# martingoe/physics

Measured on AMD Instinct MI355X. Metric: rigid_body_steps_per_sec, higher is better.
Workload: dtype f32; 1 GPU; C5_256000_tower; n_bodies=256000, bodies_per_gpu=256000, dt_nanos=16666667, preroll_steps=30, rccl_ranks=0

## Files before the change

include/spec/contact_solve.h:

```cpp
#ifndef PHYS_SPEC_CONTACT_SOLVE_H
#define PHYS_SPEC_CONTACT_SOLVE_H

#include "collide.h"

#define PHYS_MAX_COLORS 64
#define PHYS_COLOR_CACHE_PERIOD 64
#define PHYS_WARM_DIST 0.05f
#define PHYS_WARM_DOT 0.999f

typedef struct {
    float dt;
    float baumgarte;
    float slop;
    float friction;
    float max_bias;
} solve_params_t;

typedef struct {
    v3 rA, rB;
    float normal_mass;
    float tangent_mass[2];
    float bias;
    float pn;
    float pt[2];
// ... 253 lines not shown
            }
        }
    }
}

typedef struct {
    v3 n, t1, t2;
    int count;
    int has_b;
    v3 pt[4];
    float bias[4];
    float pn[4], pt0[4], pt1[4];
    float mass[4][3];
} geo_manifold_t;

PHYS_HD void solve_manifold_geo(geo_manifold_t* gm, int make_masses, int apply_only, float friction, v3 xA, float invMA, const m33* IA,
                                v3 xB, float invMB, const m33* IB, v3* vA, v3* wA, v3* vB, v3* wB) {
    const v3 zero = v3_make(0.0f, 0.0f, 0.0f);
    const int has_b = gm->has_b;
    v3 lA[3], lB[3];
    PHYS_UNROLL
    for (int d = 0; d < 3; ++d) {
        const v3 dir = d == 0 ? gm->t1 : (d == 1 ? gm->t2 : gm->n);
        lA[d] = v3_scale(dir, invMA);
        lB[d] = has_b ? v3_scale(dir, invMB) : zero;
    }
    PHYS_UNROLL
    for (int k = 0; k < 4; ++k) {
        if (k < gm->count) {
            const v3 rA = v3_sub(gm->pt[k], xA);
            const v3 rB = has_b ? v3_sub(gm->pt[k], xB) : zero;
            PHYS_UNROLL
            for (int t = 0; t < 3; ++t) {
                const v3 dir = t == 0 ? gm->t1 : (t == 1 ? gm->t2 : gm->n);
                jac_row_t j;
                j.aA = v3_cross_f(rA, dir);
                j.mA = inertia_mul(IA, j.aA);
                if (has_b) {
                    j.aB = v3_cross_f(rB, dir);
                    j.mB = inertia_mul(IB, j.aB);
                } else {
                    j.aB = zero; j.mB = zero;
                }
                if (make_masses) {
                    float km = invMA + v3_dot_f(j.mA, j.aA);
                    if (has_b) km = (km + invMB) + v3_dot_f(j.mB, j.aB);
                    gm->mass[k][t] = km > 0.0f ? 1.0f / km : 0.0f;
                }
                if (apply_only) {
                    row_apply(t == 0 ? gm->pt0[k] : (t == 1 ? gm->pt1[k] : gm->pn[k]), lA[t], lB[t], &j, has_b, vA, wA, vB, wB);
                    continue;
                }
                const float mass = gm->mass[k][t];
                const float vrel = row_velocity(dir, &j, has_b, *vA, *wA, *vB, *wB);
                float lambda;
                if (t < 2) {
                    float* acc = t == 0 ? &gm->pt0[k] : &gm->pt1[k];
                    lambda = -mass * vrel;
                    const float maxf = friction * gm->pn[k];
                    const float old = *acc;
                    const float np = det_maxf(-maxf, det_minf(old + lambda, maxf));
                    lambda = np - old;
                    *acc = np;
                } else {
                    lambda = mass * (gm->bias[k] - vrel);
                    const float old = gm->pn[k];
                    const float np = det_maxf(old + lambda, 0.0f);
                    lambda = np - old;
                    gm->pn[k] = np;
                }
                row_apply(lambda, lA[t], lB[t], &j, has_b, vA, wA, vB, wB);
            }
        }
    }
}

#endif
```

physics_amd/csrc/abi.hip:

```cpp
#include <algorithm>
#include <atomic>
#include <cmath>
#include <cstdlib>
#include <cstring>
#include <limits>
#include <string>
#include <vector>

#include "kernels.hpp"

namespace phys {
static thread_local std::string g_error;
void set_error(const std::string& msg) { g_error = msg; }
const char* get_error() { return g_error.c_str(); }
}

using namespace phys;

namespace phys {
void poll_snapshots(phys_world* w);
StepCounters* snapshot_acquire(phys_world* w) {
    const uint32_t k = w->snap_next;
    if (w->snap_pending[k]) {
        (void)hipEventSynchronize(w->snap_event[k]);
// ... 449 lines not shown

static int32_t fetch_counters(phys_world* w) {
    PHYS_HIP_TRY(hipMemcpyAsync(w->h_counters, w->counters.p, sizeof(StepCounters), hipMemcpyDeviceToHost, w->stream));
    PHYS_HIP_TRY(hipStreamSynchronize(w->stream));
    return PHYS_OK;
}

int32_t phys_sync(phys_world* w) {
    ENTER(w);
    const int32_t rc = fetch_counters(w);
    if (rc != PHYS_OK) return rc;
    poll_snapshots(w);
    const uint32_t bits = w->h_counters->overflow | w->h_counters->sticky_overflow | w->host_sticky_overflow;
    if (w->h_counters->n_static_pairs > w->static_pairs_seen) w->static_pairs_seen = w->h_counters->n_static_pairs;
    w->host_sticky_overflow = 0;
    if (w->h_counters->sticky_overflow) {
        PHYS_HIP_TRY(hipMemsetAsync(&w->counters.p->sticky_overflow, 0, sizeof(uint32_t), w->stream));
        PHYS_HIP_TRY(hipStreamSynchronize(w->stream));
    }
    if (bits & kOvfCorruptRow) {
        const uint32_t* g = w->h_counters->debug;
        return fail(PHYS_ERR_HIP, ("internal error: a solver row names no body of this world and was refused (row " +
                                   std::to_string(g[0]) + ": a " + std::to_string(g[1]) + ", b " + std::to_string(g[2]) + ", points " +
                                   std::to_string(g[3]) + "; colour " + std::to_string(g[6]) + " rows [" + std::to_string(g[4]) + ", " +
                                   std::to_string(g[5]) + "), tile base " + std::to_string(g[7]) + ")").c_str());
    }
    if (w->h_counters->debug[0] != 0u) {
        PHYS_HIP_TRY(hipMemsetAsync(w->counters.p->debug, 0, sizeof(w->counters.p->debug), w->stream));
        PHYS_HIP_TRY(hipStreamSynchronize(w->stream));
    }
    if ((bits & kOvfHandoff) && w->h_counters->debug[0] == 0xC1u) {
        const uint32_t* g = w->h_counters->debug;
        return fail(PHYS_ERR_HIP, ("contact solver hand-off timed out (k_solve_cluster) in a step since the last phys_sync; velocities "
                                   "are invalid from that step on. First lane to give up: cluster " + std::to_string(g[1] & 0xFFFFu) + " of " + std::to_string(g[1] >> 16) + ", row " +
                                   std::to_string(g[2]) + ", bodies " + std::to_string(g[3]) + " / " + std::to_string(g[4]) +
                                   ", tickets " + std::to_string(g[5] & 0xFFFFu) + " / " + std::to_string(g[5] >> 16) + ", waiting A/B " +
                                   std::to_string(g[6] & 1u) + "/" + std::to_string((g[6] >> 1) & 1u) + ", modes " +
                                   std::to_string((g[6] >> 4) & 3u) + "/" + std::to_string((g[6] >> 8) & 3u) + ", iteration " +
                                   std::to_string((g[7] >> 8) & 0xFFu) + ", colour " + std::to_string(g[7] & 0xFFu) +
                                   ". If other work shares this GPU with phys_update, create the world WITHOUT PHYS_FLAG_EXCLUSIVE_GPU").c_str());
    }
    if (bits & kOvfHandoff)
        return fail(PHYS_ERR_HIP, "contact solver hand-off timed out (k_solve_flow) in a step since the last phys_sync; "
                                  "velocities are invalid from that step on");
    if (bits & kOvfColors)
        return fail(PHYS_ERR_CAPACITY, "a body has more than 64 contact manifolds (PHYS_MAX_COLORS): the contact solve of "
                                       "that step was skipped. This limit is not configurable");
    if (bits & kOvfHalo)
        return fail(PHYS_ERR_CAPACITY, "halo record / cross-pair capacity exceeded in a step since the last phys_sync");
    if (bits & kOvfColorTable)
        return fail(PHYS_ERR_CAPACITY, "the persistent colour table is full (a look-up or an insert gave up after thousands of "
                                       "slots): the contact solve of that step was skipped. Raise phys_config.max_manifolds");
    if (bits)
        return fail(PHYS_ERR_CAPACITY, "pair / manifold capacity exceeded in a step since the last phys_sync (the contact "
                                       "solve of that step was skipped): raise phys_config.max_pairs / max_manifolds");
    return PHYS_OK;
}

static int32_t d2h(phys_world* w, void* dst, const void* src, size_t bytes) {
// ... 506 lines not shown
```

physics_amd/csrc/cluster.hip:

```cpp
#include <algorithm>
#include <cstdio>
#include <cstdlib>
#include <mutex>
#include <vector>

#include "kernels.hpp"

namespace phys {

constexpr int kClusterPerCuDiag = 3, kClusterPerCuFull = 2;
constexpr size_t kClusterLdsPerCu = 160 * 1024;
constexpr size_t kClusterSlotBytesDecl = 64;
size_t cluster_lds_bytes(uint32_t slots);

__host__ __device__ __forceinline__ uint32_t side_info(uint32_t slot, uint32_t mode) { return (slot & 0x3FFFu) | (mode << 14); }

static uint32_t spread10(uint32_t x) {
    x &= 0x3ffu;
    x = (x ^ (x << 16)) & 0xff0000ffu;
    x = (x ^ (x << 8)) & 0x0300f00fu;
    x = (x ^ (x << 4)) & 0x030c30c3u;
    x = (x ^ (x << 2)) & 0x09249249u;
    return x;
}

static size_t seg_count_offset(uint64_t n) { return ((size_t)2 * n + 3) & ~(size_t)3; }

static uint32_t clusters_on_chip(int per_cu, int cus) { return (uint32_t)std::max(8, per_cu * (cus - cus / 8)); }

int32_t cluster_assign(phys_world* w, const float* pos ) {
    w->cluster_count = 0;
    w->seg_count_dirty = false;
    w->seg_count_bins = 0;
    const uint64_t n = w->n, n_owned = w->n_owned;
    const DebugSwitches& dbg = debug_switches();
    w->cluster_dynamic = false;
    w->cluster_homes_valid = false;
    if (dbg.no_cluster || n_owned < kClusterMinBodies || !w->flow_vel.p) return PHYS_OK;
    int cus = 0;
    PHYS_HIP_TRY(hipDeviceGetAttribute(&cus, hipDeviceAttributeMultiprocessorCount, w->device));
    w->cluster_cus = cus;
    const int per_cu_max = w->all_diag_inertia ? kClusterPerCuDiag : kClusterPerCuFull;
    int per_cu = dbg.clusters_per_cu ? std::min(per_cu_max, std::max(1, *dbg.clusters_per_cu)) : per_cu_max;
    uint32_t slots = 0;
    bool fits = !dbg.cluster_dynamic;
    for (; fits; --per_cu) {
        const uint32_t max_clusters = clusters_on_chip(per_cu, cus);
        slots = (uint32_t)((n_owned + max_clusters - 1) / max_clusters);
        slots = (slots + 63u) / 64u * 64u;
        const size_t per_wg = (cluster_lds_bytes(slots) + 1023) / 1024 * 1024;
        if (per_wg * (size_t)per_cu <= kClusterLdsPerCu && slots <= kClusterMaxSlots) break;
        if (per_cu == 1) fits = false;
    }
    if (!fits) {
        const uint32_t clusters_max = clusters_on_chip(per_cu_max, cus);
        const size_t homes_max = (size_t)cus * (kClusterLdsPerCu / kClusterSlotBytesDecl) + 64;
        PHYS_HIP_TRY(w->cluster_slot.resize(n));
        PHYS_HIP_TRY(w->cluster_body.resize(homes_max));
        PHYS_HIP_TRY(w->body_shared.resize(seg_count_offset(n) + (size_t)clusters_max * PHYS_MAX_COLORS + 4));
        PHYS_HIP_TRY(hipMemsetAsync(w->body_shared.p, 0, (seg_count_offset(n) + (size_t)clusters_max * PHYS_MAX_COLORS + 4) * 4, w->stream));
        PHYS_HIP_TRY(w->seg_start.resize((size_t)clusters_max * PHYS_MAX_COLORS + 4));
        PHYS_HIP_TRY(w->man_rank.resize(w->max_manifolds));
        PHYS_HIP_TRY(w->active_flag.resize(n + 4));
        PHYS_HIP_TRY(w->active_rank.resize(n + 4));
        w->cluster_dynamic = true;
        w->cluster_count = 0;
// ... 35 lines not shown
    w->cluster_count = clusters;
    w->cluster_slots = slots;
    return PHYS_OK;
}

bool cluster_plan_dynamic(phys_world* w) {
    if (!w->cluster_dynamic) return false;
    if (!w->sorted_grid_valid) return false;
    if (w->cluster_homes_valid && w->cluster_age < kClusterDynamicPeriod) return true;
    w->cluster_homes_valid = false;
    uint64_t active = w->hint.n_active;
    if (active == 0) active = std::min<uint64_t>(w->n_owned, (uint64_t)w->hint.n_manifolds);
    if (active == 0) return false;
    const DebugSwitches& dbg = debug_switches();
    const int per_cu_max = w->all_diag_inertia ? kClusterPerCuDiag : kClusterPerCuFull;
    int per_cu = dbg.clusters_per_cu ? std::min(per_cu_max, std::max(1, *dbg.clusters_per_cu)) : per_cu_max;
    const int cus = w->cluster_cus;
    uint64_t want = active + active / 4;
    if (dbg.cluster_cap && want > dbg.cluster_cap) want = dbg.cluster_cap;
    for (;; --per_cu) {
        const uint32_t clusters = clusters_on_chip(per_cu, cus);
        uint32_t slots = (uint32_t)((want + clusters - 1) / clusters);
        slots = std::max(64u, (slots + 63u) / 64u * 64u);
        const size_t per_wg = (cluster_lds_bytes(slots) + 1023) / 1024 * 1024;
        const bool ok = per_wg * (size_t)per_cu <= kClusterLdsPerCu && slots <= kClusterMaxSlots;
        if (ok || per_cu == 1) {
            if ((!ok || per_cu < per_cu_max) && !dbg.cluster_cap && !dbg.clusters_per_cu) return false;
            if (!ok && !dbg.cluster_cap) return false;
            if (!ok) slots = kClusterMaxSlots / 64u * 64u;
            w->cluster_count = clusters;
            w->cluster_slots = slots;
            return true;
        }
    }
}

__device__ __forceinline__ uint32_t bucket_order(uint32_t i, const uint32_t* __restrict__ bucket_of, const uint32_t* __restrict__ rank,
                                                 const uint32_t* __restrict__ bucket_start) {
    const uint32_t bk = bucket_of[i];
    return bk == 0xFFFFFFFFu ? 0xFFFFFFFFu : bucket_start[bk] + rank[i];
}
__global__ __launch_bounds__(256) void k_active_flags(uint32_t n_owned, const unsigned long long* __restrict__ used,
// ... 126 lines not shown
    uint32_t* seg_count = w->body_shared.p + seg_count_offset(w->n);
    (void)hipMemsetAsync(w->body_shared.p, 0, self_zeroing ? (size_t)w->n * 8 : (seg_count_offset(w->n) + (size_t)std::max<uint32_t>(bins, w->seg_count_bins)) * 4, s);
    w->seg_count_bins = bins;
    const uint64_t key_trips = w->hint.valid ? ((uint64_t)w->hint.n_manifolds * 5 / 4) / (256u * kKeysItems) + 1 : blocks;
    const unsigned key_blocks = (unsigned)std::min<uint64_t>(blocks, std::max<uint64_t>(1, key_trips));
    hipLaunchKernelGGL(k_cluster_keys, dim3(key_blocks), dim3(256), 0, s, w->max_manifolds, w->man_a.p, w->man_b.p, w->man_color.p,
                       w->cluster_slot.p, w->cluster_slots, w->cluster_count, seg_count, w->man_rank.p, w->body_shared.p, w->counters.p);
    launch_exclusive_scan(w, seg_count, bins, w->seg_start.p, scan_is_one_launch(bins));
    hipLaunchKernelGGL(k_cluster_place, dim3(blocks), dim3(256), 0, s, w->max_manifolds, w->man_a.p, w->man_b.p, w->man_color.p,
                       w->cluster_slot.p, w->cluster_slots, w->cluster_count, w->seg_start.p, w->man_rank.p, w->row_src.p, w->counters.p, snap_out);
}

struct ClusterRowArrays { float4* all; uint64_t cap; };
constexpr int kClusterPlaneHdr = 0, kClusterPlaneN = 1, kClusterPlaneGeo = 2, kClusterPlaneAcc = 6, kClusterPlaneMass = 9, kClusterPlaneForeign = 12;
constexpr uint32_t kClusterSlotBytes = 64;
size_t cluster_lds_bytes(uint32_t slots) { return (size_t)slots * kClusterSlotBytes + (PHYS_MAX_COLORS + 1) * 4 + 12; }

constexpr int kClusterThreads = 256;
#ifndef PHYS_POLL_SLEEP
#define PHYS_POLL_SLEEP 8
#endif
constexpr int kPollSleep = PHYS_POLL_SLEEP;
template <bool DIAG, bool GUARDED, bool MAT>
__global__ __launch_bounds__(kClusterThreads, DIAG ? kClusterPerCuDiag : kClusterPerCuFull) void k_solve_cluster(StepCounters* ctr, uint32_t iterations, uint32_t epoch,
                                                                  ClusterRowArrays rows, float friction,
                                                                  const float* __restrict__ inv_inertia, uint32_t inertia_stride,
                                                                  float* vel, const float* __restrict__ pos, float* flow_vel, uint32_t n_bodies,
                                                                  const uint32_t* __restrict__ cluster_body,
                                                                  const uint32_t* __restrict__ body_shared,
                                                                  const uint32_t* __restrict__ seg_start, uint32_t slots,
                                                                  long long timeout_ticks, uint32_t attempt,
                                                                  uint32_t last_attempt, long long arrive_ticks,
                                                                  uint32_t warm_sweep , const uint32_t* __restrict__ row_src,
                                                                  float* __restrict__ man_imp ) {
    extern __shared__ __attribute__((aligned(16))) float4 s_lds[];
    float4* s_body = s_lds;
    uint32_t* s_seg = reinterpret_cast<uint32_t*>(s_lds + 4 * (size_t)slots);
    if (ctr->overflow) return;
    if (GUARDED && attempt != 0u && ctr->cluster_state[attempt - 1u] == 1u) return;
    const uint32_t cluster = blockIdx.x;
    const uint32_t n_colors = ctr->n_colors;
    const uint32_t etag = epoch << 16;
    const size_t cap = (size_t)rows.cap;
    const __amdgpu_buffer_rsrc_t rv = __builtin_amdgcn_make_buffer_rsrc(flow_vel, 0, n_bodies * 32u, 0x00020000);
    for (uint32_t sl = threadIdx.x; sl < slots; sl += kClusterThreads) {
        const uint32_t body = cluster_body[(size_t)cluster * slots + sl];
        float4 a = make_float4(0.0f, 0.0f, 0.0f, __uint_as_float(etag)), b = make_float4(0.0f, 0.0f, 0.0f, 0.0f), c = b, e = b;
        if (body != 0xFFFFFFFFu) {
            const float4 v0 = reinterpret_cast<const float4*>(vel)[2 * (size_t)body];
            const float4 v1 = reinterpret_cast<const float4*>(vel)[2 * (size_t)body + 1];
            const v3 x = ld3(pos, body);
            a = make_float4(v0.x, v0.y, v0.z, __uint_as_float(etag));
// ... 50 lines not shown
        const float4* row = rows.all + d;
        hraw = row[kClusterPlaneHdr * cap];
        nn = row[kClusterPlaneN * cap];
        fb = row[kClusterPlaneForeign * cap];
        if (DIAG) fi = row[(kClusterPlaneForeign + 1) * cap];
#pragma unroll
        for (int k = 0; k < 4; ++k) geo[k] = row[(kClusterPlaneGeo + k) * cap];
#pragma unroll
        for (int k = 0; k < 3; ++k) {
            acc[k] = make_float4(0.0f, 0.0f, 0.0f, 0.0f);
            mas[k] = acc[k];
            if (lit != 0u || warm_sweep != 0u) acc[k] = row[(kClusterPlaneAcc + k) * cap];
            if (lit != 0u) mas[k] = row[(kClusterPlaneMass + k) * cap];
        }
    };
    hraw = make_float4(0.0f, 0.0f, 0.0f, 0.0f); nn = hraw; fb = hraw; fi = hraw;
#pragma unroll
    for (int k = 0; k < 4; ++k) geo[k] = hraw;
#pragma unroll
    for (int k = 0; k < 3; ++k) { acc[k] = hraw; mas[k] = hraw; }
    if (have) fetch();
    uint32_t it = 0, col = 0;
    for (uint32_t step = 0; step < steps; ++step) {
        const bool last_it = it + 1 == iterations;
        {
            const uint32_t seg_hi = s_seg[col + 1];
            while (have && lit == it && d < seg_hi) {
                const uint32_t d_row = d;
                const uint32_t hw = __float_as_uint(hraw.w);
                const uint4 h = MAT ? make_uint4(__float_as_uint(hraw.x), __float_as_uint(hraw.y), ((hw >> 6) & 3u) | ((hw >> 13) & 4u), hw & 0xFFFF7F3Fu)
                                    : make_uint4(__float_as_uint(hraw.x), __float_as_uint(hraw.y), __float_as_uint(hraw.z), hw);
                const uint32_t info = __float_as_uint(nn.w);
                const uint32_t modeA = (info >> 14) & 3u, modeB = (info >> 30) & 3u;
                const uint32_t slotA = info & 0x1FFFu, slotB = (info >> 16) & 0x1FFFu;
                const bool pubA = (info >> 13) & 1u, pubB = (info >> 29) & 1u;
                geo_manifold_t gm;
                gm.count = (int)h.z;
                gm.has_b = !PHYS_IS_STATIC_PARTNER(h.y);
                gm.n = v3_make(nn.x, nn.y, nn.z);
                tangent_basis(gm.n, &gm.t1, &gm.t2);
                {
                    const float flat[12] = {acc[0].x, acc[0].y, acc[0].z, acc[0].w, acc[1].x, acc[1].y, acc[1].z, acc[1].w,
                                            acc[2].x, acc[2].y, acc[2].z, acc[2].w};
                    const float flam[12] = {mas[0].x, mas[0].y, mas[0].z, mas[0].w, mas[1].x, mas[1].y, mas[1].z, mas[1].w,
                                            mas[2].x, mas[2].y, mas[2].z, mas[2].w};
#pragma unroll
                    for (int k = 0; k < 4; ++k) {
                        gm.pt[k] = v3_make(geo[k].x, geo[k].y, geo[k].z);
                        gm.bias[k] = geo[k].w;
                        gm.pn[k] = flat[3 * k]; gm.pt0[k] = flat[3 * k + 1]; gm.pt1[k] = flat[3 * k + 2];
                        gm.mass[k][0] = flam[3 * k]; gm.mass[k][1] = flam[3 * k + 1]; gm.mass[k][2] = flam[3 * k + 2];
                    }
                }
                const uint32_t rankA = h.w & 0xFFu, degA = (h.w >> 8) & 0xFFu, rankB = (h.w >> 16) & 0xFFu, degB = h.w >> 24;
                const uint32_t tA = it * degA + rankA, tB = it * degB + rankB;
                const bool finalA = last_it && rankA + 1 == degA, finalB = last_it && rankB + 1 == degB;
                v3 vA, wA, xA, vB = v3_make(0.0f, 0.0f, 0.0f), wB = vB, xB = vB;
                float ima, imb = 0.0f;
                bool needA = false, needB = false;
                m33 IA, IB;
#pragma unroll
                for (int k = 0; k < 9; ++k) { IA.m[k] = 0.0f; IB.m[k] = 0.0f; }
                v3 vA0 = v3_make(0.0f, 0.0f, 0.0f);
                vA = vA0; wA = vA0; xA = vA0; ima = 0.0f;
                if (modeA == 0u || modeA == 1u) {
                    const float4* sa = s_body + 4 * slotA;
                    const float4 la = sa[0], lb = sa[1], lc = sa[2];
                    vA = v3_make(la.x, la.y, la.z); wA = v3_make(lb.x, lb.y, lb.z); ima = lb.w;
// ... 16 lines not shown
                    vB = v3_make(la.x, la.y, la.z); wB = v3_make(lb.x, lb.y, lb.z); imb = lb.w;
                    xB = v3_make(lc.x, lc.y, lc.z);
                    if (DIAG) { const float4 li = sb[3]; IB.m[0] = li.x; IB.m[4] = li.y; IB.m[8] = li.z; }
                    if (modeB == 1u) needB = __float_as_uint(la.w) != (etag | tB);
                } else if (modeB == 2u) {
                    xB = v3_make(fb.x, fb.y, fb.z); imb = fb.w;
                    if (DIAG) { IB.m[0] = fi.x; IB.m[4] = fi.y; IB.m[8] = fi.z; }
                    if (tB == 0u) {
                        const BodyVel B0 = ld_vel(vel, h.y);
                        vB = B0.v; wB = B0.w;
                    }
                    needB = tB != 0u;
                }
                if (!DIAG) {
                    IA = ld_inertia<false>(inv_inertia, h.x * inertia_stride);
                    if (gm.has_b) IB = ld_inertia<false>(inv_inertia, h.y * inertia_stride);
                }
                uint32_t sweeps = 0, late = 0;
                while (needA || needB) {
                    if (needA) {
                        const u32x4 g0 = ld_granule(rv, h.x * 32u), g1 = ld_granule(rv, h.x * 32u + 16u);
                        if (g0.w == (etag | tA) && g1.w == (etag | tA)) { vA = granule_v3(g0); wA = granule_v3(g1); needA = false; }
                    }
                    if (needB) {
                        const u32x4 g0 = ld_granule(rv, h.y * 32u), g1 = ld_granule(rv, h.y * 32u + 16u);
                        if (g0.w == (etag | tB) && g1.w == (etag | tB)) { vB = granule_v3(g0); wB = granule_v3(g1); needB = false; }
                    }
                    if (needA || needB) {
                        __builtin_amdgcn_s_sleep(kPollSleep);
                        if ((++sweeps & 63u) == 0u) {
                            const bool gone = (wall_clock64() - t_start > timeout_ticks) ||
// ... 1 lines not shown
                            if (gone) {
                                late = (needA ? 1u : 0u) | (needB ? 2u : 0u);
                                flag_overflow(ctr, kOvfHandoff); dead = true; needA = false; needB = false;
                            }
                        }
                    }
                }
                if (GUARDED && late && atomicCAS(&ctr->debug[0], 0u, 0xC1u) == 0u) {
                    ctr->debug[1] = cluster | (gridDim.x << 16);
                    ctr->debug[2] = d_row; ctr->debug[3] = h.x; ctr->debug[4] = h.y;
                    ctr->debug[5] = (tA & 0xFFFFu) | (tB << 16);
                    ctr->debug[6] = late | (modeA << 4) | (modeB << 8);
                    ctr->debug[7] = (col & 0xFFu) | ((it & 0xFFu) << 8);
                }
                if (!dead) {
                    solve_manifold_geo(&gm, it == 0u, (warm_sweep != 0u && it == 0u) ? 1 : 0, MAT ? hraw.z : friction, xA, ima, &IA, xB, imb, &IB, &vA, &wA, &vB, &wB);
                    if (modeA == 0u || modeA == 1u) {
                        s_body[4 * slotA] = make_float4(vA.x, vA.y, vA.z, __uint_as_float(etag | (tA + 1u)));
                        s_body[4 * slotA + 1] = make_float4(wA.x, wA.y, wA.z, ima);
                    }
                    if (modeA == 1u || modeA == 2u) {
                        if (finalA) { st3(vel + 8 * (size_t)h.x, 0, vA); st3(vel + 8 * (size_t)h.x + 4, 0, wA); }
                        else if (modeA == 2u || pubA) { st_granule(rv, h.x * 32u, vA, etag | (tA + 1u)); st_granule(rv, h.x * 32u + 16u, wA, etag | (tA + 1u)); }
                    }
                    if (modeB == 0u || modeB == 1u) {
                        s_body[4 * slotB] = make_float4(vB.x, vB.y, vB.z, __uint_as_float(etag | (tB + 1u)));
                        s_body[4 * slotB + 1] = make_float4(wB.x, wB.y, wB.z, imb);
                    }
                    if (modeB == 1u || modeB == 2u) {
                        if (finalB) { st3(vel + 8 * (size_t)h.y, 0, vB); st3(vel + 8 * (size_t)h.y + 4, 0, wB); }
                        else if (modeB == 2u || pubB) { st_granule(rv, h.y * 32u, vB, etag | (tB + 1u)); st_granule(rv, h.y * 32u + 16u, wB, etag | (tB + 1u)); }
                    }
                    if (last_it && man_imp) {
                        float4* o = reinterpret_cast<float4*>(man_imp) + 3 * (size_t)row_src[d_row];
                        o[0] = make_float4(gm.pn[0], gm.pt0[0], gm.pt1[0], gm.pn[1]);
                        o[1] = make_float4(gm.pt0[1], gm.pt1[1], gm.pn[2], gm.pt0[2]);
                        o[2] = make_float4(gm.pt1[2], gm.pn[3], gm.pt0[3], gm.pt1[3]);
                    }
                    if (!last_it) {
                        float4* out = rows.all + d_row;
                        out[(kClusterPlaneAcc + 0) * cap] = make_float4(gm.pn[0], gm.pt0[0], gm.pt1[0], gm.pn[1]);
                        if (gm.count > 1) out[(kClusterPlaneAcc + 1) * cap] = make_float4(gm.pt0[1], gm.pt1[1], gm.pn[2], gm.pt0[2]);
                        if (gm.count > 2) out[(kClusterPlaneAcc + 2) * cap] = make_float4(gm.pt1[2], gm.pn[3], gm.pt0[3], gm.pt1[3]);
                        if (it == 0u) {
                            out[(kClusterPlaneMass + 0) * cap] = make_float4(gm.mass[0][0], gm.mass[0][1], gm.mass[0][2], gm.mass[1][0]);
                            if (gm.count > 1) out[(kClusterPlaneMass + 1) * cap] = make_float4(gm.mass[1][1], gm.mass[1][2], gm.mass[2][0], gm.mass[2][1]);
                            if (gm.count > 2) out[(kClusterPlaneMass + 2) * cap] = make_float4(gm.mass[2][2], gm.mass[3][0], gm.mass[3][1], gm.mass[3][2]);
                        }
                    }
                }
                d += kClusterThreads;
                if (d >= row_end) {
                    d = row_base + threadIdx.x; ++lit;
                    if (d == d_row) asm volatile("s_waitcnt vmcnt(0)" ::: "memory");
                }
                have = lit < iterations && !dead;
                if (have) fetch();
            }
            if (seg_hi != s_seg[col]) asm volatile("s_waitcnt lgkmcnt(0)\n\ts_barrier" ::: "memory");
        }
        if (++col == n_colors) { col = 0u; ++it; }
    }
    for (uint32_t sl = threadIdx.x; sl < slots; sl += kClusterThreads) {
        const uint32_t body = cluster_body[(size_t)cluster * slots + sl];
        if (body == 0xFFFFFFFFu || (body_shared[2 * (size_t)body] | body_shared[2 * (size_t)body + 1])) continue;
        const float4 a = s_body[4 * sl], b = s_body[4 * sl + 1];
        st3(vel + 8 * (size_t)body, 0, v3_make(a.x, a.y, a.z));
        st3(vel + 8 * (size_t)body + 4, 0, v3_make(b.x, b.y, b.z));
    }
}

void launch_solve_cluster(phys_world* w, void* row_all, uint64_t cap, float friction, const float* inertia, uint32_t stride,
                          bool diag, long long timeout_ticks, bool materials) {
    const uint32_t warm_sweep = w->warm ? 1u : 0u;
    const uint32_t sweeps = w->cfg.solver_iterations + warm_sweep;
    ClusterRowArrays rows;
    rows.all = (float4*)row_all; rows.cap = cap;
    const size_t lds = cluster_lds_bytes(w->cluster_slots);
    const dim3 g(w->cluster_count), b(kClusterThreads);
    static std::mutex chain_lock;
    static hipEvent_t chain_event[64] = {};
    std::lock_guard<std::mutex> hold(chain_lock);
    {
        static bool attr_set[64] = {};
        if (!attr_set[w->device & 63]) {
            hipError_t e = hipSuccess;
            auto allow = [&](const void* f) { if (e == hipSuccess) e = hipFuncSetAttribute(f, hipFuncAttributeMaxDynamicSharedMemorySize, 160 * 1024); };
            allow(reinterpret_cast<const void*>(&k_solve_cluster<true, true, false>)); allow(reinterpret_cast<const void*>(&k_solve_cluster<true, false, false>));
            allow(reinterpret_cast<const void*>(&k_solve_cluster<false, true, false>)); allow(reinterpret_cast<const void*>(&k_solve_cluster<false, false, false>));
            allow(reinterpret_cast<const void*>(&k_solve_cluster<true, true, true>)); allow(reinterpret_cast<const void*>(&k_solve_cluster<true, false, true>));
            allow(reinterpret_cast<const void*>(&k_solve_cluster<false, true, true>)); allow(reinterpret_cast<const void*>(&k_solve_cluster<false, false, true>));
            if (e != hipSuccess) { (void)hipGetLastError(); set_error(std::string("hipFuncSetAttribute(k_solve_cluster): ") + hipGetErrorString(e)); }
            else attr_set[w->device & 63] = true;
        }
    }
    hipEvent_t& ev = chain_event[w->device & 63];
    if (ev) (void)hipStreamWaitEvent(w->stream, ev, 0);
    else (void)hipEventCreateWithFlags(&ev, hipEventDisableTiming);
    struct Record { hipEvent_t e; hipStream_t s; ~Record() { if (e) (void)hipEventRecord(e, s); } } record{ev, w->stream};
    const bool guarded = !gpu_is_exclusive(w);
    dispatch_bool(diag, [&](auto diag_t) { dispatch_bool(guarded, [&](auto guarded_t) { dispatch_bool(materials, [&](auto mat_t) {
        constexpr bool D = decltype(diag_t)::value, G = decltype(guarded_t)::value, MT = decltype(mat_t)::value;
        const uint32_t kAttempts = G ? 2u : 1u;
        for (uint32_t attempt = 0; attempt < kAttempts; ++attempt) {
            const uint32_t last = attempt + 1 == kAttempts ? 1u : 0u;
            const long long arrive_ticks = !G ? -1ll : (attempt == 0 ? 50000ll : 2000000ll);
            hipLaunchKernelGGL((k_solve_cluster<D, G, MT>), g, b, lds, w->stream, w->counters.p, sweeps, w->flow_epoch, rows, friction,
                               inertia, stride, w->vel.p, w->pos.p, w->flow_vel.p, (uint32_t)w->n, w->cluster_body.p,
                               w->body_shared.p, w->seg_start.p, w->cluster_slots, timeout_ticks, attempt, last, arrive_ticks,
                               warm_sweep, w->row_src.p, w->warm ? w->man_imp.p : (float*)nullptr);
// ... 6 lines not shown
```

physics_amd/csrc/solver.hip:

```cpp
#include <cstdlib>

#include "kernels.hpp"

namespace phys {

struct WarmJob {
    const uint32_t* man_prev;
    const float* geo_prev;
    const float* imp_prev;
    float* imp;
    const uint32_t* row_src;
};
__device__ __forceinline__ void store_final_impulses(const WarmJob& wj, uint32_t d, const float pn[4], const float pt0[4], const float pt1[4]) {
    float4* o = reinterpret_cast<float4*>(wj.imp) + 3 * (size_t)wj.row_src[d];
    o[0] = make_float4(pn[0], pt0[0], pt1[0], pn[1]);
    o[1] = make_float4(pt0[1], pt1[1], pn[2], pt0[2]);
    o[2] = make_float4(pt1[2], pn[3], pt0[3], pt1[3]);
}

struct RowArrays {
    float4* all;
    uint4* hdr;
    float4* n;
    float4* pt;
// ... 893 lines not shown
    mats.body = reinterpret_cast<const float2*>(w->mat.p);
    mats.st = reinterpret_cast<const float2*>(w->st_mat.p);
    mats.ground = make_float2(w->ground_mat_set ? w->ground_mat[0] : w->cfg.friction, w->ground_mat_set ? w->ground_mat[1] : 0.0f);
    mats.threshold = w->restitution_threshold;
    dispatch_bool(diag, [&](auto diag_t) { dispatch_bool(materials, [&](auto mat_t) {
        constexpr bool DIAG = decltype(diag_t)::value, MAT = decltype(mat_t)::value;
        { PHYS_PROF(w, PHYS_STAGE_ROWS);
          auto rows_build = [&](auto... mat) {
              hipLaunchKernelGGL((k_rows_build<DIAG, MAT, decltype(mat)...>), grid_for_count(m_hint), tb, 0, s, w->counters.p, rows, sp, w->row_src.p, w->man_geo.p,
                                 w->pos.p, w->vel.p, inertia, stride, w->man_color.p,
                                 w->color_state.p, flow ? (stall ? 2 : 1) : 0, table, w->cluster_slot.p, w->body_shared.p,
                                 w->cluster_step ? w->cluster_slots : 0u, w->cluster_count, warm, mat...);
          };
          if constexpr (MAT) rows_build(mats); else rows_build(); }
        if (flow) {
            if (cluster) {
                PHYS_PROF(w, PHYS_STAGE_SOLVE_CLUSTER);
                launch_solve_cluster(w, rows.all, cap, sp.friction, inertia, stride, diag, timeout_ticks, MAT);
                return;
            }
            const bool quad = m_hint <= (dbg.flow_quad_max ? dbg.flow_quad_max : (w->flow_wide ? kFlowMaxManifolds : kFlowQuadMaxManifolds));
            const uint32_t threads = 256u;
            const uint32_t rows_per_item = quad ? threads / 4 : threads;
            uint64_t items = (uint64_t)sweeps * ((m_hint * 5 / 4 + rows_per_item - 1) / rows_per_item) + 1;
            int cus = 256;
            (void)hipDeviceGetAttribute(&cus, hipDeviceAttributeMultiprocessorCount, w->device);
            const uint64_t most = quad ? (w->flow_wide && m_hint > 32768u ? (uint64_t)(3 * (cus - cus / 8)) : 224) : 256;
            if (items > most) items = most;
            PHYS_PROF(w, PHYS_STAGE_SOLVE_FLOW);
            const uint64_t per_color = m_hint / (h.valid && h.n_colors ? h.n_colors : 1u);
// ... 45 lines not shown
```

physics_amd/csrc/world.hpp:

```cpp
#pragma once
#include <hip/hip_runtime.h>

#include <cstddef>
#include <cstdint>
#include <optional>
#include <string>
#include <vector>

#include "../../include/physics_hip.h"

namespace phys {

constexpr int kMaxColors = 64;
constexpr uint64_t kClusterMinBodies = 32768;
constexpr uint32_t kClusterDynamicPeriod = 8;
constexpr uint64_t kClusterMinManifolds = 170000;
constexpr uint64_t kFlowWideMaxManifolds = 400000;
constexpr uint32_t kClusterMaxSlots = 2496;

void set_error(const std::string& msg);
const char* get_error();

#define PHYS_HIP_TRY(expr)                                                                          \
    do {                                                                                            \
// ... 168 lines not shown

struct phys_world {
    ~phys_world();
    phys_config cfg;
    int device = 0;
    hipStream_t stream = nullptr;
    uint64_t n = 0;
    uint64_t n_owned = 0;
    uint64_t max_ghosts = 0;
    float slab_lo = -3.0e38f, slab_hi = 3.0e38f, slab_reach = 0.0f;
    phys::DevBuf<uint32_t> halo_block_counts;
    uint64_t steps = 0;
    bool forces_dirty = false;
    bool singular_inertia = false;
    bool all_diag_inertia = true;
    bool uniform_inertia = true;
    bool body_capsules = false;
    bool aabbs_valid = false;
    bool grid_valid = false;

    phys::DevBuf<float> pos, rot, vel , force, torque, inv_inertia, inv_inertia_diag , half_extent, aabb;
    phys::DevBuf<uint32_t> shape;
    phys::DevBuf<uint32_t> global_id;
    phys::DevBuf<float> geo;
    phys::DevBuf<uint32_t> filt;
    bool body_filters_set = false;
    bool static_filters_set = false;
    bool ground_filter_set = false;
    uint32_t ground_filt = 0xFFFF0001u;
    phys::DevBuf<float> mat, st_mat;
// ... 124 lines not shown
```

Measured before the change: 212.8 million body-steps/s.

## Park manifold registers in LDS to cut cluster-solver register pressure

Splits the manifold solve into a per-point routine and drops the geo_manifold_t struct copy in k_solve_cluster. In the diagonal-inertia variant it parks two float4 row values (the fourth contact point and the last mass plane) in a per-thread LDS area, to lower VGPR pressure. Cluster planning now asks the occupancy API whether a given number of clusters per CU can really be resident, and adds a per-CU value of 4 that only debug switches can reach; the default plan stays at 3. It also reports which solver kernel timed out on hand-off; the cost is extra LDS per workgroup and LDS round trips inside the inner solve.

```diff
diff --git a/include/spec/contact_solve.h b/include/spec/contact_solve.h
--- a/include/spec/contact_solve.h
+++ b/include/spec/contact_solve.h
@@ -291,64 +291,64 @@
     float mass[4][3];
 } geo_manifold_t;
 
+PHYS_HD void solve_point_geo(v3 n, v3 t1, v3 t2, int has_b, v3 pt, float bias, float* pn, float* pt0, float* pt1, float* mass ,
+                             int make_masses, int apply_only, float friction, v3 xA, float invMA, const m33* IA, v3 xB, float invMB,
+                             const m33* IB, v3* vA, v3* wA, v3* vB, v3* wB) {
+    const v3 zero = v3_make(0.0f, 0.0f, 0.0f);
+    const v3 rA = v3_sub(pt, xA);
+    const v3 rB = has_b ? v3_sub(pt, xB) : zero;
+    PHYS_UNROLL
+    for (int t = 0; t < 3; ++t) {
+        const v3 dir = t == 0 ? t1 : (t == 1 ? t2 : n);
+        const v3 lA = v3_scale(dir, invMA);
+        const v3 lB = has_b ? v3_scale(dir, invMB) : zero;
+        jac_row_t j;
+        j.aA = v3_cross_f(rA, dir);
+        j.mA = inertia_mul(IA, j.aA);
+        if (has_b) {
+            j.aB = v3_cross_f(rB, dir);
+            j.mB = inertia_mul(IB, j.aB);
+        } else {
+            j.aB = zero; j.mB = zero;
+        }
+        if (make_masses) {
+            float km = invMA + v3_dot_f(j.mA, j.aA);
+            if (has_b) km = (km + invMB) + v3_dot_f(j.mB, j.aB);
+            mass[t] = km > 0.0f ? 1.0f / km : 0.0f;
+        }
+        if (apply_only) {
+            row_apply(t == 0 ? *pt0 : (t == 1 ? *pt1 : *pn), lA, lB, &j, has_b, vA, wA, vB, wB);
+            continue;
+        }
+        const float m = mass[t];
+        const float vrel = row_velocity(dir, &j, has_b, *vA, *wA, *vB, *wB);
+        float lambda;
+        if (t < 2) {
+            float* acc = t == 0 ? pt0 : pt1;
+            lambda = -m * vrel;
+            const float maxf = friction * *pn;
+            const float old = *acc;
+            const float np = det_maxf(-maxf, det_minf(old + lambda, maxf));
+            lambda = np - old;
+            *acc = np;
+        } else {
+            lambda = m * (bias - vrel);
+            const float old = *pn;
+            const float np = det_maxf(old + lambda, 0.0f);
+            lambda = np - old;
+            *pn = np;
+        }
+        row_apply(lambda, lA, lB, &j, has_b, vA, wA, vB, wB);
+    }
+}
+
 PHYS_HD void solve_manifold_geo(geo_manifold_t* gm, int make_masses, int apply_only, float friction, v3 xA, float invMA, const m33* IA,
                                 v3 xB, float invMB, const m33* IB, v3* vA, v3* wA, v3* vB, v3* wB) {
-    const v3 zero = v3_make(0.0f, 0.0f, 0.0f);
-    const int has_b = gm->has_b;
-    v3 lA[3], lB[3];
-    PHYS_UNROLL
-    for (int d = 0; d < 3; ++d) {
-        const v3 dir = d == 0 ? gm->t1 : (d == 1 ? gm->t2 : gm->n);
-        lA[d] = v3_scale(dir, invMA);
-        lB[d] = has_b ? v3_scale(dir, invMB) : zero;
-    }
-    PHYS_UNROLL
-    for (int k = 0; k < 4; ++k) {
-        if (k < gm->count) {
-            const v3 rA = v3_sub(gm->pt[k], xA);
-            const v3 rB = has_b ? v3_sub(gm->pt[k], xB) : zero;
-            PHYS_UNROLL
-            for (int t = 0; t < 3; ++t) {
-                const v3 dir = t == 0 ? gm->t1 : (t == 1 ? gm->t2 : gm->n);
-                jac_row_t j;
-                j.aA = v3_cross_f(rA, dir);
-                j.mA = inertia_mul(IA, j.aA);
-                if (has_b) {
-                    j.aB = v3_cross_f(rB, dir);
-                    j.mB = inertia_mul(IB, j.aB);
-                } else {
-                    j.aB = zero; j.mB = zero;
-                }
-                if (make_masses) {
-                    float km = invMA + v3_dot_f(j.mA, j.aA);
-                    if (has_b) km = (km + invMB) + v3_dot_f(j.mB, j.aB);
-                    gm->mass[k][t] = km > 0.0f ? 1.0f / km : 0.0f;
-                }
-                if (apply_only) {
-                    row_apply(t == 0 ? gm->pt0[k] : (t == 1 ? gm->pt1[k] : gm->pn[k]), lA[t], lB[t], &j, has_b, vA, wA, vB, wB);
-                    continue;
-                }
-                const float mass = gm->mass[k][t];
-                const float vrel = row_velocity(dir, &j, has_b, *vA, *wA, *vB, *wB);
-                float lambda;
-                if (t < 2) {
-                    float* acc = t == 0 ? &gm->pt0[k] : &gm->pt1[k];
-                    lambda = -mass * vrel;
-                    const float maxf = friction * gm->pn[k];
-                    const float old = *acc;
-                    const float np = det_maxf(-maxf, det_minf(old + lambda, maxf));
-                    lambda = np - old;
-                    *acc = np;
-                } else {
-                    lambda = mass * (gm->bias[k] - vrel);
-                    const float old = gm->pn[k];
-                    const float np = det_maxf(old + lambda, 0.0f);
-                    lambda = np - old;
-                    gm->pn[k] = np;
-                }
-                row_apply(lambda, lA[t], lB[t], &j, has_b, vA, wA, vB, wB);
-            }
-        }
+    PHYS_UNROLL
+    for (int k = 0; k < 4; ++k) {
+        if (k < gm->count)
+            solve_point_geo(gm->n, gm->t1, gm->t2, gm->has_b, gm->pt[k], gm->bias[k], &gm->pn[k], &gm->pt0[k], &gm->pt1[k], gm->mass[k],
+                            make_masses, apply_only, friction, xA, invMA, IA, xB, invMB, IB, vA, wA, vB, wB);
     }
 }
 
diff --git a/physics_amd/csrc/abi.hip b/physics_amd/csrc/abi.hip
--- a/physics_amd/csrc/abi.hip
+++ b/physics_amd/csrc/abi.hip
@@ -487,6 +487,8 @@
     const uint32_t bits = w->h_counters->overflow | w->h_counters->sticky_overflow | w->host_sticky_overflow;
     if (w->h_counters->n_static_pairs > w->static_pairs_seen) w->static_pairs_seen = w->h_counters->n_static_pairs;
     w->host_sticky_overflow = 0;
+    const uint32_t handoff_kernels = w->handoff_kernels;
+    w->handoff_kernels = 0;
     if (w->h_counters->sticky_overflow) {
         PHYS_HIP_TRY(hipMemsetAsync(&w->counters.p->sticky_overflow, 0, sizeof(uint32_t), w->stream));
         PHYS_HIP_TRY(hipStreamSynchronize(w->stream));
@@ -514,8 +516,9 @@
                                    ". If other work shares this GPU with phys_update, create the world WITHOUT PHYS_FLAG_EXCLUSIVE_GPU").c_str());
     }
     if (bits & kOvfHandoff)
-        return fail(PHYS_ERR_HIP, "contact solver hand-off timed out (k_solve_flow) in a step since the last phys_sync; "
-                                  "velocities are invalid from that step on");
+        return fail(PHYS_ERR_HIP, (std::string("contact solver hand-off timed out (") +
+                                   (handoff_kernels == 2u ? "k_solve_cluster" : handoff_kernels == 1u ? "k_solve_flow" : "k_solve_cluster or k_solve_flow") +
+                                   ") in a step since the last phys_sync; velocities are invalid from that step on").c_str());
     if (bits & kOvfColors)
         return fail(PHYS_ERR_CAPACITY, "a body has more than 64 contact manifolds (PHYS_MAX_COLORS): the contact solve of "
                                        "that step was skipped. This limit is not configurable");
diff --git a/physics_amd/csrc/cluster.hip b/physics_amd/csrc/cluster.hip
--- a/physics_amd/csrc/cluster.hip
+++ b/physics_amd/csrc/cluster.hip
@@ -1,17 +1,24 @@
 #include <algorithm>
 #include <cstdio>
 #include <cstdlib>
+#include <map>
 #include <mutex>
+#include <tuple>
 #include <vector>
 
 #include "kernels.hpp"
 
 namespace phys {
 
-constexpr int kClusterPerCuDiag = 3, kClusterPerCuFull = 2;
+constexpr int kClusterPerCuDiag = 4, kClusterPerCuDiagMin = 3, kClusterPerCuFull = 2;
 constexpr size_t kClusterLdsPerCu = 160 * 1024;
 constexpr size_t kClusterSlotBytesDecl = 64;
-size_t cluster_lds_bytes(uint32_t slots);
+size_t cluster_lds_bytes(uint32_t slots, bool diag);
+static int cluster_resident_per_cu(const phys_world* w, size_t lds);
+static bool cluster_plan_resident(const phys_world* w, int per_cu, uint32_t slots) {
+    if (per_cu <= (w->all_diag_inertia ? kClusterPerCuDiagMin : kClusterPerCuFull)) return true;
+    return cluster_resident_per_cu(w, cluster_lds_bytes(slots, w->all_diag_inertia)) >= per_cu;
+}
 
 __host__ __device__ __forceinline__ uint32_t side_info(uint32_t slot, uint32_t mode) { return (slot & 0x3FFFu) | (mode << 14); }
 
@@ -41,15 +48,16 @@
     PHYS_HIP_TRY(hipDeviceGetAttribute(&cus, hipDeviceAttributeMultiprocessorCount, w->device));
     w->cluster_cus = cus;
     const int per_cu_max = w->all_diag_inertia ? kClusterPerCuDiag : kClusterPerCuFull;
-    int per_cu = dbg.clusters_per_cu ? std::min(per_cu_max, std::max(1, *dbg.clusters_per_cu)) : per_cu_max;
+    const int per_cu_plan = w->all_diag_inertia ? kClusterPerCuDiagMin : kClusterPerCuFull;
+    int per_cu = dbg.clusters_per_cu ? std::min(per_cu_max, std::max(1, *dbg.clusters_per_cu)) : per_cu_plan;
     uint32_t slots = 0;
     bool fits = !dbg.cluster_dynamic;
     for (; fits; --per_cu) {
         const uint32_t max_clusters = clusters_on_chip(per_cu, cus);
         slots = (uint32_t)((n_owned + max_clusters - 1) / max_clusters);
         slots = (slots + 63u) / 64u * 64u;
-        const size_t per_wg = (cluster_lds_bytes(slots) + 1023) / 1024 * 1024;
-        if (per_wg * (size_t)per_cu <= kClusterLdsPerCu && slots <= kClusterMaxSlots) break;
+        const size_t per_wg = (cluster_lds_bytes(slots, w->all_diag_inertia) + 1023) / 1024 * 1024;
+        if (per_wg * (size_t)per_cu <= kClusterLdsPerCu && slots <= kClusterMaxSlots && cluster_plan_resident(w, per_cu, slots)) break;
         if (per_cu == 1) fits = false;
     }
     if (!fits) {
@@ -115,7 +123,8 @@
     if (active == 0) return false;
     const DebugSwitches& dbg = debug_switches();
     const int per_cu_max = w->all_diag_inertia ? kClusterPerCuDiag : kClusterPerCuFull;
-    int per_cu = dbg.clusters_per_cu ? std::min(per_cu_max, std::max(1, *dbg.clusters_per_cu)) : per_cu_max;
+    const int per_cu_plan = w->all_diag_inertia ? kClusterPerCuDiagMin : kClusterPerCuFull;
+    int per_cu = dbg.clusters_per_cu ? std::min(per_cu_max, std::max(1, *dbg.clusters_per_cu)) : per_cu_plan;
     const int cus = w->cluster_cus;
     uint64_t want = active + active / 4;
     if (dbg.cluster_cap && want > dbg.cluster_cap) want = dbg.cluster_cap;
@@ -123,10 +132,10 @@
         const uint32_t clusters = clusters_on_chip(per_cu, cus);
         uint32_t slots = (uint32_t)((want + clusters - 1) / clusters);
         slots = std::max(64u, (slots + 63u) / 64u * 64u);
-        const size_t per_wg = (cluster_lds_bytes(slots) + 1023) / 1024 * 1024;
-        const bool ok = per_wg * (size_t)per_cu <= kClusterLdsPerCu && slots <= kClusterMaxSlots;
+        const size_t per_wg = (cluster_lds_bytes(slots, w->all_diag_inertia) + 1023) / 1024 * 1024;
+        const bool ok = per_wg * (size_t)per_cu <= kClusterLdsPerCu && slots <= kClusterMaxSlots && cluster_plan_resident(w, per_cu, slots);
         if (ok || per_cu == 1) {
-            if ((!ok || per_cu < per_cu_max) && !dbg.cluster_cap && !dbg.clusters_per_cu) return false;
+            if ((!ok || per_cu < per_cu_plan) && !dbg.cluster_cap && !dbg.clusters_per_cu) return false;
             if (!ok && !dbg.cluster_cap) return false;
             if (!ok) slots = kClusterMaxSlots / 64u * 64u;
             w->cluster_count = clusters;
@@ -283,9 +292,13 @@
 struct ClusterRowArrays { float4* all; uint64_t cap; };
 constexpr int kClusterPlaneHdr = 0, kClusterPlaneN = 1, kClusterPlaneGeo = 2, kClusterPlaneAcc = 6, kClusterPlaneMass = 9, kClusterPlaneForeign = 12;
 constexpr uint32_t kClusterSlotBytes = 64;
-size_t cluster_lds_bytes(uint32_t slots) { return (size_t)slots * kClusterSlotBytes + (PHYS_MAX_COLORS + 1) * 4 + 12; }
-
 constexpr int kClusterThreads = 256;
+constexpr size_t kClusterSegBytes = (PHYS_MAX_COLORS + 1) * 4 + 12;
+static_assert(kClusterSegBytes % 16 == 0, "the parked planes behind the segment table are float4");
+constexpr int kClusterParkPlanes = 2;
+size_t cluster_lds_bytes(uint32_t slots, bool diag) {
+    return (size_t)slots * kClusterSlotBytes + kClusterSegBytes + (diag ? (size_t)kClusterParkPlanes * kClusterThreads * 16 : 0);
+}
 #ifndef PHYS_POLL_SLEEP
 #define PHYS_POLL_SLEEP 8
 #endif
@@ -305,6 +318,8 @@
     extern __shared__ __attribute__((aligned(16))) float4 s_lds[];
     float4* s_body = s_lds;
     uint32_t* s_seg = reinterpret_cast<uint32_t*>(s_lds + 4 * (size_t)slots);
+    constexpr bool PARK = DIAG;
+    float4* s_park = s_lds + 4 * (size_t)slots + kClusterSegBytes / 16;
     if (ctr->overflow) return;
     if (GUARDED && attempt != 0u && ctr->cluster_state[attempt - 1u] == 1u) return;
     const uint32_t cluster = blockIdx.x;
@@ -385,12 +400,14 @@
             if (lit != 0u) mas[k] = row[(kClusterPlaneMass + k) * cap];
         }
     };
-    hraw = make_float4(0.0f, 0.0f, 0.0f, 0.0f); nn = hraw; fb = hraw; fi = hraw;
-#pragma unroll
-    for (int k = 0; k < 4; ++k) geo[k] = hraw;
-#pragma unroll
-    for (int k = 0; k < 3; ++k) { acc[k] = hraw; mas[k] = hraw; }
-    if (have) fetch();
+    auto no_row = [&]() {
+        hraw = make_float4(0.0f, 0.0f, 0.0f, 0.0f); nn = hraw; fb = hraw; fi = hraw;
+#pragma unroll
+        for (int k = 0; k < 4; ++k) geo[k] = hraw;
+#pragma unroll
+        for (int k = 0; k < 3; ++k) { acc[k] = hraw; mas[k] = hraw; }
+    };
+    if (have) fetch(); else no_row();
     uint32_t it = 0, col = 0;
     for (uint32_t step = 0; step < steps; ++step) {
         const bool last_it = it + 1 == iterations;
@@ -405,24 +422,20 @@
                 const uint32_t modeA = (info >> 14) & 3u, modeB = (info >> 30) & 3u;
                 const uint32_t slotA = info & 0x1FFFu, slotB = (info >> 16) & 0x1FFFu;
                 const bool pubA = (info >> 13) & 1u, pubB = (info >> 29) & 1u;
-                geo_manifold_t gm;
-                gm.count = (int)h.z;
-                gm.has_b = !PHYS_IS_STATIC_PARTNER(h.y);
-                gm.n = v3_make(nn.x, nn.y, nn.z);
-                tangent_basis(gm.n, &gm.t1, &gm.t2);
-                {
-                    const float flat[12] = {acc[0].x, acc[0].y, acc[0].z, acc[0].w, acc[1].x, acc[1].y, acc[1].z, acc[1].w,
-                                            acc[2].x, acc[2].y, acc[2].z, acc[2].w};
-                    const float flam[12] = {mas[0].x, mas[0].y, mas[0].z, mas[0].w, mas[1].x, mas[1].y, mas[1].z, mas[1].w,
-                                            mas[2].x, mas[2].y, mas[2].z, mas[2].w};
-#pragma unroll
-                    for (int k = 0; k < 4; ++k) {
-                        gm.pt[k] = v3_make(geo[k].x, geo[k].y, geo[k].z);
-                        gm.bias[k] = geo[k].w;
-                        gm.pn[k] = flat[3 * k]; gm.pt0[k] = flat[3 * k + 1]; gm.pt1[k] = flat[3 * k + 2];
-                        gm.mass[k][0] = flam[3 * k]; gm.mass[k][1] = flam[3 * k + 1]; gm.mass[k][2] = flam[3 * k + 2];
-                    }
-                }
+                float4* const park = s_park + threadIdx.x;
+                if (PARK) {
+                    park[0 * kClusterThreads] = geo[3]; park[1 * kClusterThreads] = mas[2];
+                    asm volatile("" ::: "memory");
+                }
+                const int count = (int)h.z;
+                const int has_b = !PHYS_IS_STATIC_PARTNER(h.y);
+                const v3 rn = v3_make(nn.x, nn.y, nn.z);
+                v3 rt1, rt2;
+                tangent_basis(rn, &rt1, &rt2);
+                float pn[4] = {acc[0].x, acc[0].w, acc[1].z, acc[2].y}, pt0[4] = {acc[0].y, acc[1].x, acc[1].w, acc[2].z},
+                      pt1[4] = {acc[0].z, acc[1].y, acc[2].x, acc[2].w};
+                float ms[4][3] = {{mas[0].x, mas[0].y, mas[0].z}, {mas[0].w, mas[1].x, mas[1].y}, {mas[1].z, mas[1].w, 0.0f}, {0.0f, 0.0f, 0.0f}};
+                if (!PARK) { ms[2][2] = mas[2].x; ms[3][0] = mas[2].y; ms[3][1] = mas[2].z; ms[3][2] = mas[2].w; }
                 const uint32_t rankA = h.w & 0xFFu, degA = (h.w >> 8) & 0xFFu, rankB = (h.w >> 16) & 0xFFu, degB = h.w >> 24;
                 const uint32_t tA = it * degA + rankA, tB = it * degB + rankB;
                 const bool finalA = last_it && rankA + 1 == degA, finalB = last_it && rankB + 1 == degB;
@@ -469,7 +482,7 @@
                 }
                 if (!DIAG) {
                     IA = ld_inertia<false>(inv_inertia, h.x * inertia_stride);
-                    if (gm.has_b) IB = ld_inertia<false>(inv_inertia, h.y * inertia_stride);
+                    if (has_b) IB = ld_inertia<false>(inv_inertia, h.y * inertia_stride);
                 }
                 uint32_t sweeps = 0, late = 0;
                 while (needA || needB) {
@@ -501,7 +514,21 @@
                     ctr->debug[7] = (col & 0xFFu) | ((it & 0xFFu) << 8);
                 }
                 if (!dead) {
-                    solve_manifold_geo(&gm, it == 0u, (warm_sweep != 0u && it == 0u) ? 1 : 0, MAT ? hraw.z : friction, xA, ima, &IA, xB, imb, &IB, &vA, &wA, &vB, &wB);
+#pragma unroll
+                    for (int k = 0; k < 4; ++k) {
+                        if (k < count) {
+                            float4 g = geo[k];
+                            float ia = ima, ib = imb;
+                            if (PARK) {
+                                asm volatile("" ::: "memory");
+                                if (k == 3) g = park[0 * kClusterThreads];
+                                if (k == 2) { const float4 m2 = park[1 * kClusterThreads]; ms[2][2] = m2.x; ms[3][0] = m2.y; ms[3][1] = m2.z; ms[3][2] = m2.w; }
+                                asm volatile("" : "+v"(ia), "+v"(ib));
+                            }
+                            solve_point_geo(rn, rt1, rt2, has_b, v3_make(g.x, g.y, g.z), g.w, &pn[k], &pt0[k], &pt1[k], ms[k], it == 0u,
+                                            (warm_sweep != 0u && it == 0u) ? 1 : 0, MAT ? hraw.z : friction, xA, ia, &IA, xB, ib, &IB, &vA, &wA, &vB, &wB);
+                        }
+                    }
                     if (modeA == 0u || modeA == 1u) {
                         s_body[4 * slotA] = make_float4(vA.x, vA.y, vA.z, __uint_as_float(etag | (tA + 1u)));
                         s_body[4 * slotA + 1] = make_float4(wA.x, wA.y, wA.z, ima);
@@ -520,19 +547,19 @@
                     }
                     if (last_it && man_imp) {
                         float4* o = reinterpret_cast<float4*>(man_imp) + 3 * (size_t)row_src[d_row];
-                        o[0] = make_float4(gm.pn[0], gm.pt0[0], gm.pt1[0], gm.pn[1]);
-                        o[1] = make_float4(gm.pt0[1], gm.pt1[1], gm.pn[2], gm.pt0[2]);
-                        o[2] = make_float4(gm.pt1[2], gm.pn[3], gm.pt0[3], gm.pt1[3]);
+                        o[0] = make_float4(pn[0], pt0[0], pt1[0], pn[1]);
+                        o[1] = make_float4(pt0[1], pt1[1], pn[2], pt0[2]);
+                        o[2] = make_float4(pt1[2], pn[3], pt0[3], pt1[3]);
                     }
                     if (!last_it) {
                         float4* out = rows.all + d_row;
-                        out[(kClusterPlaneAcc + 0) * cap] = make_float4(gm.pn[0], gm.pt0[0], gm.pt1[0], gm.pn[1]);
-                        if (gm.count > 1) out[(kClusterPlaneAcc + 1) * cap] = make_float4(gm.pt0[1], gm.pt1[1], gm.pn[2], gm.pt0[2]);
-                        if (gm.count > 2) out[(kClusterPlaneAcc + 2) * cap] = make_float4(gm.pt1[2], gm.pn[3], gm.pt0[3], gm.pt1[3]);
+                        out[(kClusterPlaneAcc + 0) * cap] = make_float4(pn[0], pt0[0], pt1[0], pn[1]);
+                        if (count > 1) out[(kClusterPlaneAcc + 1) * cap] = make_float4(pt0[1], pt1[1], pn[2], pt0[2]);
+                        if (count > 2) out[(kClusterPlaneAcc + 2) * cap] = make_float4(pt1[2], pn[3], pt0[3], pt1[3]);
                         if (it == 0u) {
-                            out[(kClusterPlaneMass + 0) * cap] = make_float4(gm.mass[0][0], gm.mass[0][1], gm.mass[0][2], gm.mass[1][0]);
-                            if (gm.count > 1) out[(kClusterPlaneMass + 1) * cap] = make_float4(gm.mass[1][1], gm.mass[1][2], gm.mass[2][0], gm.mass[2][1]);
-                            if (gm.count > 2) out[(kClusterPlaneMass + 2) * cap] = make_float4(gm.mass[2][2], gm.mass[3][0], gm.mass[3][1], gm.mass[3][2]);
+                            out[(kClusterPlaneMass + 0) * cap] = make_float4(ms[0][0], ms[0][1], ms[0][2], ms[1][0]);
+                            if (count > 1) out[(kClusterPlaneMass + 1) * cap] = make_float4(ms[1][1], ms[1][2], ms[2][0], ms[2][1]);
+                            if (count > 2) out[(kClusterPlaneMass + 2) * cap] = make_float4(ms[2][2], ms[3][0], ms[3][1], ms[3][2]);
                         }
                     }
                 }
@@ -542,7 +569,7 @@
                     if (d == d_row) asm volatile("s_waitcnt vmcnt(0)" ::: "memory");
                 }
                 have = lit < iterations && !dead;
-                if (have) fetch();
+                if (have) fetch(); else no_row();
             }
             if (seg_hi != s_seg[col]) asm volatile("s_waitcnt lgkmcnt(0)\n\ts_barrier" ::: "memory");
         }
@@ -557,30 +584,60 @@
     }
 }
 
+static const void* const kClusterKernels[2][2][2] = {
+    {{reinterpret_cast<const void*>(&k_solve_cluster<false, false, false>), reinterpret_cast<const void*>(&k_solve_cluster<false, false, true>)},
+     {reinterpret_cast<const void*>(&k_solve_cluster<false, true, false>), reinterpret_cast<const void*>(&k_solve_cluster<false, true, true>)}},
+    {{reinterpret_cast<const void*>(&k_solve_cluster<true, false, false>), reinterpret_cast<const void*>(&k_solve_cluster<true, false, true>)},
+     {reinterpret_cast<const void*>(&k_solve_cluster<true, true, false>), reinterpret_cast<const void*>(&k_solve_cluster<true, true, true>)}}};
+
+static bool cluster_kernels_allow_lds(int device) {
+    static std::mutex lock;
+    static bool attr_set[64] = {};
+    std::lock_guard<std::mutex> hold(lock);
+    if (attr_set[device & 63]) return true;
+    hipError_t e = hipSuccess;
+    for (int i = 0; i < 8 && e == hipSuccess; ++i)
+        e = hipFuncSetAttribute(kClusterKernels[i >> 2][(i >> 1) & 1][i & 1], hipFuncAttributeMaxDynamicSharedMemorySize, (int)kClusterLdsPerCu);
+    if (e != hipSuccess) { (void)hipGetLastError(); set_error(std::string("hipFuncSetAttribute(k_solve_cluster): ") + hipGetErrorString(e)); return false; }
+    attr_set[device & 63] = true;
+    return true;
+}
+
+static int cluster_resident_per_cu(const phys_world* w, size_t lds) {
+    struct Key { int device, diag; size_t kib; bool operator<(const Key& o) const { return std::tie(device, diag, kib) < std::tie(o.device, o.diag, o.kib); } };
+    static std::mutex lock;
+    static std::map<Key, int> known;
+    if (!cluster_kernels_allow_lds(w->device)) return 0;
+    const int diag = w->all_diag_inertia ? 1 : 0;
+    const Key key{w->device, diag, (lds + 1023) / 1024};
+    std::lock_guard<std::mutex> hold(lock);
+    const auto at = known.find(key);
+    if (at != known.end()) return at->second;
+    int least = 1 << 30;
+    for (int i = 0; i < 4; ++i) {
+        int n = 0;
+        if (hipOccupancyMaxActiveBlocksPerMultiprocessor(&n, kClusterKernels[diag][i >> 1][i & 1], kClusterThreads, key.kib * 1024) != hipSuccess) {
+            (void)hipGetLastError();
+            n = 0;
+        }
+        least = std::min(least, n);
+    }
+    known[key] = least;
+    return least;
+}
+
 void launch_solve_cluster(phys_world* w, void* row_all, uint64_t cap, float friction, const float* inertia, uint32_t stride,
                           bool diag, long long timeout_ticks, bool materials) {
     const uint32_t warm_sweep = w->warm ? 1u : 0u;
     const uint32_t sweeps = w->cfg.solver_iterations + warm_sweep;
     ClusterRowArrays rows;
     rows.all = (float4*)row_all; rows.cap = cap;
-    const size_t lds = cluster_lds_bytes(w->cluster_slots);
+    const size_t lds = cluster_lds_bytes(w->cluster_slots, diag);
     const dim3 g(w->cluster_count), b(kClusterThreads);
     static std::mutex chain_lock;
     static hipEvent_t chain_event[64] = {};
     std::lock_guard<std::mutex> hold(chain_lock);
-    {
-        static bool attr_set[64] = {};
-        if (!attr_set[w->device & 63]) {
-            hipError_t e = hipSuccess;
-            auto allow = [&](const void* f) { if (e == hipSuccess) e = hipFuncSetAttribute(f, hipFuncAttributeMaxDynamicSharedMemorySize, 160 * 1024); };
-            allow(reinterpret_cast<const void*>(&k_solve_cluster<true, true, false>)); allow(reinterpret_cast<const void*>(&k_solve_cluster<true, false, false>));
-            allow(reinterpret_cast<const void*>(&k_solve_cluster<false, true, false>)); allow(reinterpret_cast<const void*>(&k_solve_cluster<false, false, false>));
-            allow(reinterpret_cast<const void*>(&k_solve_cluster<true, true, true>)); allow(reinterpret_cast<const void*>(&k_solve_cluster<true, false, true>));
-            allow(reinterpret_cast<const void*>(&k_solve_cluster<false, true, true>)); allow(reinterpret_cast<const void*>(&k_solve_cluster<false, false, true>));
-            if (e != hipSuccess) { (void)hipGetLastError(); set_error(std::string("hipFuncSetAttribute(k_solve_cluster): ") + hipGetErrorString(e)); }
-            else attr_set[w->device & 63] = true;
-        }
-    }
+    (void)cluster_kernels_allow_lds(w->device);
     hipEvent_t& ev = chain_event[w->device & 63];
     if (ev) (void)hipStreamWaitEvent(w->stream, ev, 0);
     else (void)hipEventCreateWithFlags(&ev, hipEventDisableTiming);
diff --git a/physics_amd/csrc/solver.hip b/physics_amd/csrc/solver.hip
--- a/physics_amd/csrc/solver.hip
+++ b/physics_amd/csrc/solver.hip
@@ -931,6 +931,7 @@
           };
           if constexpr (MAT) rows_build(mats); else rows_build(); }
         if (flow) {
+            w->handoff_kernels |= cluster ? 2u : 1u;
             if (cluster) {
                 PHYS_PROF(w, PHYS_STAGE_SOLVE_CLUSTER);
                 launch_solve_cluster(w, rows.all, cap, sp.friction, inertia, stride, diag, timeout_ticks, MAT);
diff --git a/physics_amd/csrc/world.hpp b/physics_amd/csrc/world.hpp
--- a/physics_amd/csrc/world.hpp
+++ b/physics_amd/csrc/world.hpp
@@ -206,6 +206,7 @@
     bool forces_dirty = false;
     bool singular_inertia = false;
     bool all_diag_inertia = true;
+    uint32_t handoff_kernels = 0;
     bool uniform_inertia = true;
     bool body_capsules = false;
     bool aabbs_valid = false;
```

New measurement: 191.1 million body-steps/s. 10.2% lower.
